# HadrienG2/grayscott

Hardware: AMD Instinct MI355X
Metric: Mcells×steps/s and achieved HBM GB/s (% of roofline), 16384² f32 grid (higher is better)
Workload: dtype f32

## Files before the change

### grayscott_amd/capi.py

```python
from __future__ import annotations

import ctypes
import os

_HERE = os.path.dirname(os.path.abspath(__file__))
LIB_PATH = os.environ.get("GS_HIP_LIBRARY") or os.path.join(_HERE, "libgs_hip.so")

GS_OK = 0
GS_ERR_INVALID = -1
GS_ERR_HIP = -2
GS_ERR_RCCL = -3
GS_ERR_NO_DEVICE = -4
GS_ERR_UNSUPPORTED = -5
GS_ERR_NOMEM = -6

GS_MATH_STRICT, GS_MATH_FUSED = 0, 1
GS_KERNEL_AUTO, GS_KERNEL_SIMPLE, GS_KERNEL_STREAM, GS_KERNEL_TB, GS_KERNEL_LDS, GS_KERNEL_TILE, GS_KERNEL_WINDOW = 0, 1, 2, 3, 4, 5, 6
GS_BOUNDARY_CLIPPED, GS_BOUNDARY_ZERO_HALO, GS_BOUNDARY_PERIODIC, GS_BOUNDARY_NEUMANN = 0, 1, 2, 3
GS_UNIQUE_ID_BYTES = 128
GS_REGION_PAIRS_MAX = 1 << 25
GS_REGION_HIST_MAX = 1 << 25
GS_REGION_SPECTRUM_MAX = 1 << 25
GS_REGION_SPECTRUM_RECORDS_MAX = 1 << 27
GS_REGION_COMPONENTS_MAX = 1 << 20
# ... 27 lines not shown
    "gs_fields_compare", "gs_members_compare", "gs_fields_copy", "gs_members_copy",
    "gs_members_set_active", "gs_members_get_active",
    "gs_members_set_noise", "gs_members_get_noise", "gs_members_clear_noise",
    "gs_fields_morphology", "gs_members_morphology",
    "gs_region_grid", "gs_fields_region_summaries", "gs_fields_region_morphology", "gs_fields_region_correlation",
    "gs_fields_region_histogram", "gs_fields_region_components", "gs_fields_region_compare", "gs_fields_region_spectrum",
    "gs_fields_correlation", "gs_members_correlation",
    "gs_spectrum_tables", "gs_fields_spectrum", "gs_members_spectrum",
    "gs_fields_components", "gs_members_components",
    "gs_field_component_list", "gs_members_component_list", "gs_component_list_view", "gs_component_list_destroy",
    "gs_fields_match", "gs_members_match", "gs_component_match_view", "gs_component_match_destroy",
    "gs_time_stats_create", "gs_time_stats_destroy", "gs_time_stats_reset", "gs_time_stats_accumulate", "gs_time_stats_samples",
    "gs_time_stats_result", "gs_time_stats_download",
    "gs_members_time_stats_create", "gs_members_time_stats_accumulate", "gs_members_time_stats_result",
    "gs_members_bundle_stats",
    "gs_ctx_quiet_stats", "gs_ctx_quiet_edge_stats",
)


class GsError(RuntimeError):

    def __init__(self, code: int, message: str):
        super().__init__(f"gs_hip error {code}: {message}")
        self.code = code
        self.message = message


class GsParams(ctypes.Structure):

    _fields_ = [
        ("w", (ctypes.c_float * 3) * 3),
# ... 157 lines not shown
        "gs_timer_start": (i32, [vp]),
        "gs_timer_stop": (i32, [vp, P(f32)]),
        "gs_ctx_info": (i32, [vp, ctypes.c_char_p, ctypes.c_size_t, P(u64)]),
        "gs_host_alloc": (i32, [P(vp), u64]),
        "gs_host_free": (i32, [vp]),
        "gs_field_download_async": (i32, [vp, vp, vp]),
        "gs_download_wait": (i32, [vp]),
        "gs_ctx_get_tuned": (i32, [vp, u64, u64, P(i32), P(i32), P(i32), P(i32)]),
        "gs_ctx_set_tuned": (i32, [vp, u64, u64, i32, i32, i32, i32]),
        "gs_ctx_comm_info": (i32, [vp, P(i32), P(i32), P(i32)]),
        "gs_field_colormap": (i32, [vp, vp, f32, vp, i32, vp]),
        "gs_ctx_stats": (i32, [vp, P(GsStats)]),
        "gs_ctx_set_pass_timing": (i32, [vp, i32]),
        "gs_ctx_quiet_stats": (i32, [vp, P(u64)]),
        "gs_ctx_quiet_edge_stats": (i32, [vp, P(u64)]),
        "gs_field_mark_written": (i32, [vp, vp]),
        "gs_rccl_selftest": (i32, [i32, u64]),
        "gs_runtime_info": (i32, [i32, ctypes.c_char_p, ctypes.c_size_t]),
        "gs_fields_place": (i32, [vp, P(vp), i32, P(f32), P(f32)]),
        "gs_debug_place_stats": (i32, [vp, P(u64), P(u64)]),
        "gs_download_wait_but": (i32, [vp, i32]),
        "gs_debug_exchange_probe_create": (i32, [i32, i32, i32, u64, P(vp)]),
        "gs_debug_exchange_probe_run": (i32, [vp, P(f32), P(f32)]),
        "gs_debug_exchange_probe_destroy": (i32, [vp]),
        "gs_ensemble_create": (i32, [vp, P(vp), u64, u64, u64]),
        "gs_ensemble_destroy": (i32, [vp, vp]),
        "gs_ensemble_shape": (i32, [vp, P(u64), P(u64), P(u64)]),
        "gs_ensemble_set_params": (i32, [vp, vp, P(GsParams), u64]),
        "gs_ensemble_seed": (i32, [vp, vp]),
        "gs_ensemble_upload": (i32, [vp, vp, u64, u64, vp, vp]),
# ... 105 lines not shown
```

### grayscott_amd/csrc/gs_api.cpp

```cpp
#include "gs_internal.h"

namespace gsi {

bool is_pow2_or_zero(float w)
{
    if (w == 0.0f) return true;
    int e = 0;
    const float m = std::frexp(std::fabs(w), &e);
    return m == 0.5f;
}

int32_t check_math(const gs_params &p, int32_t math)
{
    if (math != GS_MATH_STRICT && math != GS_MATH_FUSED)
        return fail(GS_ERR_INVALID, "unknown math flavour %d", math);
    if (math == GS_MATH_FUSED)
        for (int i = 0; i < 3; ++i)
            for (int j = 0; j < 3; ++j)
                if (!is_pow2_or_zero(p.w[i][j]))
                    return fail(GS_ERR_UNSUPPORTED,
                                "GS_MATH_FUSED needs stencil weights that are 0 or a power of two "
                                "(w[%d][%d] = %g); use GS_MATH_STRICT", i, j, (double)p.w[i][j]);
    return GS_OK;
}
// ... 169 lines not shown
                        qr.edge_skipped = sum;
                        GS_HIP(hipFree(qr.words));
                        qr.words = nullptr;
                        qr.cap = 0;
                    }
                    GS_HIP(hipMalloc(&qr.words, 3 * (size_t)q.need * sizeof(uint32_t)));
                    GS_HIP(hipMemset(qr.words, 0, 3 * (size_t)q.need * sizeof(uint32_t)));
                    qr.cap = (size_t)q.need;
                    if (!qr.skipped) {
                        GS_HIP(hipMalloc(&qr.skipped, (size_t)kQuietCounters * kQuietCounterStride * sizeof(unsigned long long)));
                        GS_HIP(hipMemset(qr.skipped, 0, (size_t)kQuietCounters * kQuietCounterStride * sizeof(unsigned long long)));
                    }
                    continue;
                }
                if (q.launched > 0) {
                    qr.launched += (uint64_t)q.launched;
                    qr.edge_launched += (uint64_t)q.edge_launched;
                    qr.passes++;
                    if (qr.mode == 3) qr.steady++;
                } else {
                    qr.refused = true;
                }
                break;
            }
            break;
        }
        e = fused ? gs_launch_tb_fused(a, fuse, stream, &name, at) : gs_launch_tb_strict(a, fuse, stream, &name, at);
        break;
    case GS_KERNEL_SIMPLE:
        e = fused ? gs_launch_simple_fused(a, stream, &name, at) : gs_launch_simple_strict(a, stream, &name, at);
// ... 443 lines not shown
                                            "set GS_RCCL_LIBRARY to the transport to use, or run one slab per process");
    }

    int ndev = 0;
    hipError_t e = hipGetDeviceCount(&ndev);
    if (e != hipSuccess || ndev == 0)
        return fail(GS_ERR_NO_DEVICE, "no HIP device available (%s)", hipGetErrorString(e));

    gs_ctx *ctx = new (std::nothrow) gs_ctx();
    if (!ctx) return fail(GS_ERR_NOMEM, "out of host memory");
    if (params) ctx->p = *params; else gs_default_params(&ctx->p);
    if (opts) ctx->o = *opts; else gs_default_options(&ctx->o);
    ctx->rank = rank;
    ctx->world = world;
    ctx->quiet.enabled = gs_env_int("GS_HIP_QUIET_UNITS", 1, 0, 1) != 0;
    int32_t st = check_math(ctx->p, ctx->o.math);
    if (st == GS_OK && ctx->o.cols_per_lane != 0 && ctx->o.cols_per_lane != 1 && ctx->o.cols_per_lane != 2 &&
        ctx->o.cols_per_lane != 4)
        st = fail(GS_ERR_INVALID, "cols_per_lane must be 0 (auto), 1, 2 or 4, not %d", ctx->o.cols_per_lane);
    if (st == GS_OK && (ctx->o.tile_shape < 0 || ctx->o.tile_shape > 3))
        st = fail(GS_ERR_INVALID, "tile_shape must be 0 (auto), 1 (32 x 64), 2 (16 x 64) or 3 (64 x 64), not %d", ctx->o.tile_shape);
    if (st == GS_OK && ctx->o.boundary != GS_BOUNDARY_CLIPPED && ctx->o.boundary != GS_BOUNDARY_ZERO_HALO &&
        ctx->o.boundary != GS_BOUNDARY_PERIODIC && ctx->o.boundary != GS_BOUNDARY_NEUMANN)
        st = fail(GS_ERR_INVALID, "unknown boundary rule %d", ctx->o.boundary);
    if (st == GS_OK && ctx->o.boundary == GS_BOUNDARY_PERIODIC) {
        if (world > 1 || n_local > 1)
            st = fail(GS_ERR_UNSUPPORTED, "the periodic boundary rule needs a single slab in a single process (got %d local "
                                          "slab(s), %d process(es))", n_local < 1 ? 1 : n_local, world);
        else if (ctx->o.kernel == GS_KERNEL_WINDOW || ctx->o.kernel == GS_KERNEL_LDS)
            st = fail(GS_ERR_UNSUPPORTED, "the periodic boundary rule has no form of the %s kernel",
// ... 77 lines not shown
}

int32_t gs_ctx_set_params(gs_ctx *ctx, const gs_params *params)
{
    if (!ctx || !params) return fail(GS_ERR_INVALID, "null argument");
    GS_TRY(check_math(*params, ctx->o.math));
    GS_TRY(resolve_window(ctx));
    ctx->p = *params;
    return GS_OK;
}

int32_t gs_step(gs_ctx *ctx, gs_field *in_u, gs_field *in_v, gs_field *out_u, gs_field *out_v)
{
    GS_TRY(check_step_fields(ctx, in_u, in_v, out_u, out_v));
    GS_TRY(check_attached_shape(ctx, in_u));
    GS_TRY(resolve_window(ctx));
    return step_impl(ctx, in_u, in_v, out_u, out_v);
}

int32_t gs_run(gs_ctx *ctx, gs_field *u0, gs_field *v0, gs_field *u1, gs_field *v1, uint64_t steps,
               int32_t *result_slot)
{
    return run_steps(ctx, u0, v0, u1, v1, steps, result_slot, true);
}

}

namespace gsi {

int32_t run_steps(gs_ctx *ctx, gs_field *u0, gs_field *v0, gs_field *u1, gs_field *v1, uint64_t steps, int32_t *result_slot,
                  bool allow_window)
{
    GS_TRY(check_step_fields(ctx, u0, v0, u1, v1));
    GS_TRY(check_attached_shape(ctx, u0));
    Run r{ctx, {u0, u1}, {v0, v1}};
    r.steps = steps;
    int fuse = 1;
    if (ctx->o.kernel == GS_KERNEL_AUTO || ctx->o.kernel == GS_KERNEL_TB || ctx->o.kernel == GS_KERNEL_TILE ||
        ctx->o.kernel == GS_KERNEL_WINDOW) {
        fuse = ctx->o.fuse_steps > 0 ? ctx->o.fuse_steps : kGhostRows;
        if (fuse > kGhostRows) fuse = kGhostRows;
        if (ctx->total_slabs() > 1 && fuse > min_slab_rows(ctx, u0)) fuse = min_slab_rows(ctx, u0);
        if (fuse < 1) fuse = 1;
    }
    const bool single = ctx->total_slabs() == 1;
    const bool mapped = ctx->attached.kind != GS_ATTACH_NONE;
    if (single && !mapped && ctx->o.kernel == GS_KERNEL_AUTO && u0->rows * u0->cols > 0 && steps > 0 &&
        u0->rows * u0->cols <= (uint64_t)kGsResidentCells) {
        SlabRt &sl = ctx->slabs[0];
// ... 81 lines not shown
    if (single && fuse > 1 && ctx->o.rows_per_block == 0 && !ctx->o.no_tune && !tuned_shape(ctx, u0, fuse))
        GS_TRY(tune_online(r, fuse));
    const int kk = tuned_shape(ctx, u0, fuse) && ctx->tuner().tuned.k > 0 && ctx->tuner().tuned.k <= fuse ? ctx->tuner().tuned.k : fuse;
    const int V = bands_for(ctx, u0, kk);
    if (ctx->o.use_graph && single && V == 1 && kk > 1) GS_TRY(replay_graph_batches(r, kk));
    gs_ctx::QuietRt &qr = ctx->quiet;
    const gs_params &pp = ctx->p;
    bool quiet = qr.enabled && single && V == 1 && !ctx->o.use_graph && !mapped && kk >= 2 && kk <= 4 &&
                 ctx->o.math == GS_MATH_STRICT && (ctx->o.boundary == GS_BOUNDARY_CLIPPED || ctx->o.boundary == GS_BOUNDARY_ZERO_HALO) &&
                 (ctx->o.kernel == GS_KERNEL_AUTO || ctx->o.kernel == GS_KERNEL_TB || ctx->o.kernel == GS_KERNEL_TILE ||
                  ctx->o.kernel == GS_KERNEL_WINDOW) &&
                 std::isfinite(pp.du) && std::isfinite(pp.dv) && std::isfinite(pp.feed) && std::isfinite(pp.kill) &&
                 std::isfinite(pp.feed + pp.kill) && std::isfinite(pp.dt);
    for (int i = 0; i < 9; ++i) quiet = quiet && std::isfinite(pp.w[i / 3][i % 3]);
    qr.refused = false;
    int quiet_pass = 0;
    const char *full_pass = nullptr;
    while (r.n < steps) {
        const int k = (steps - r.n) >= (uint64_t)kk ? kk : (int)(steps - r.n);
        if (quiet && k == kk && !qr.refused) {
            qr.mode = quiet_pass < 2 ? quiet_pass + 1 : 3;
            qr.in_slot = r.in;
            ++quiet_pass;
        }
        const int32_t st = r.advance(k == kk ? V : 1, k);
        qr.mode = 0;
        GS_TRY(st);
        if (k == kk) full_pass = ctx->last_kernel;
    }
    if (full_pass) ctx->last_kernel = full_pass;
    if (result_slot) *result_slot = r.in;
    return GS_OK;
}

}

extern "C" {

int32_t gs_sync(gs_ctx *ctx)
{
    if (!ctx) return fail(GS_ERR_INVALID, "null context");
    return sync_all(ctx);
}
// ... 93 lines not shown
int32_t gs_ctx_quiet_edge_stats(gs_ctx *ctx, uint64_t out[3])
{
    if (!ctx || !out) return fail(GS_ERR_INVALID, "null argument");
    GS_TRY(sync_all(ctx));
    out[0] = ctx->quiet.edge_launched;
    out[1] = out[2] = 0;
    if (ctx->quiet.skipped) {
        unsigned long long host[kQuietCounters * kQuietCounterStride];
        GS_HIP(hipSetDevice(ctx->slabs[0].device));
        GS_HIP(hipMemcpy(host, ctx->quiet.skipped, sizeof host, hipMemcpyDeviceToHost));
        for (int i = 0; i < kQuietCounters; ++i) out[2] += host[i * kQuietCounterStride + 2];
    }
    return gsi::quiet_edge_skips(ctx, &out[1]);
}

int32_t gs_ctx_info(const gs_ctx *ctx, char *kernel_name, size_t cap, uint64_t *launches)
{
    if (!ctx) return fail(GS_ERR_INVALID, "null context");
    if (kernel_name && cap) {
        const gs_ctx::Tuned &t = ctx->tuner().tuned;
        if (t.rpu > 0)
            std::snprintf(kernel_name, cap, "%s@%dx%d", ctx->last_kernel, t.rpu, t.split > 0 ? t.split : 1);
        else
            std::snprintf(kernel_name, cap, "%s", ctx->last_kernel);
    }
    if (launches) *launches = ctx->launches;
    return GS_OK;
}

}
// ... 1 lines not shown
```

### grayscott_amd/csrc/gs_attached.cpp

```cpp
#include "gs_internal.h"

namespace gsi {

static const char *const kKindName[GS_ATTACH_KINDS] = {"", "parameter map", "domain mask", "noise term"};
static const char *const kKindShort[GS_ATTACH_KINDS] = {"", "map", "mask", "noise"};
static const char *const kKindForm[GS_ATTACH_KINDS] = {"", "parameter-map", "domain-mask", "noise"};

static void philox2x32(uint32_t c0, uint32_t c1, uint32_t k, uint32_t out[2])
{
    for (int i = 0; i < 10; ++i) {
        const uint64_t p = (uint64_t)0xD256D193u * c0;
        c0 = (uint32_t)(p >> 32) ^ k ^ c1;
        c1 = (uint32_t)p;
        k += 0x9E3779B9u;
    }
    out[0] = c0;
    out[1] = c1;
}
uint32_t noise_key(uint64_t seed, uint64_t step)
{
    uint32_t x[2];
    philox2x32((uint32_t)step, (uint32_t)(step >> 32), (uint32_t)seed, x);
    return x[0] ^ (uint32_t)(seed >> 32);
}
// ... 58 lines not shown
    at.plane[0] = f[0];
    at.plane[1] = f[1];
    return GS_OK;
}

template <typename F>
static int32_t fill_planes(gs_ctx *ctx, gs_field *const *planes, int np, F enqueue)
{
    for (size_t i = 0; i < ctx->slabs.size(); ++i) {
        SlabRt &sl = ctx->slabs[i];
        GS_HIP(hipSetDevice(sl.device));
        GS_TRY(enqueue(i, sl, (size_t)(planes[0]->s[i].rows + 2 * kGhostRows) * planes[0]->pitch + 2 * kGuardFloats));
    }
    GS_TRY(sync_all(ctx));
    for (int j = 0; j < np; ++j) {
        planes[j]->ghost_depth = 0;
        GS_TRY(refresh_ghosts(ctx, planes[j]));
    }
    return GS_OK;
}

static int32_t copy_block(gs_field *dst, const gs_field *src, size_t i, SlabRt &sl, size_t n)
{
    GS_HIP(hipMemcpyAsync(dst->s[i].alloc, src->s[i].alloc, n * sizeof(float), hipMemcpyDeviceToDevice, sl.compute));
    return GS_OK;
}

static int32_t form_links(gs_ctx *ctx, gs_field *m)
{
    gs_field *l = ctx->attached.plane[0];
    const int32_t periodic = ctx->o.boundary == GS_BOUNDARY_PERIODIC;
// ... 92 lines not shown
```

### grayscott_amd/csrc/gs_fields.cpp

```cpp
#include <algorithm>
#include "gs_internal.h"

using namespace gsi;

namespace gsi {

int32_t plane_layout(const gs_ctx *ctx, uint64_t rows, uint64_t cols, PlaneLayout &out)
{
    const uint64_t S = (uint64_t)ctx->total_slabs();
    if (rows < S && !(rows == 0 && S == 1))
        return fail(GS_ERR_INVALID, "%llu rows cannot be split over %llu slabs",
                    (unsigned long long)rows, (unsigned long long)S);
    const int pad = ctx->o.pitch_pad > 0 ? ((ctx->o.pitch_pad + 3) / 4) * 4 : 0;
    out.pitch = (cols == 0 ? 64 : ((cols + 63) / 64) * 64) + (uint64_t)pad;
    if (out.pitch > 0x7ffffff0ull) return fail(GS_ERR_UNSUPPORTED, "too many columns");
    out.slabs.clear();
    for (size_t i = 0; i < ctx->slabs.size(); ++i) {
        const uint64_t k = (uint64_t)ctx->global_index((int)i);
        const uint64_t r0 = k * rows / S, r1 = (k + 1) * rows / S;
        if (r1 - r0 > 0x7ffffff0ull || (r1 - r0 + 2 * kGhostRows) * out.pitch > 0x7ffffff0ull * 4ull)
            return fail(GS_ERR_UNSUPPORTED, "slab too large for 32-bit row indexing");
        out.slabs.emplace_back(r0, r1 - r0);
    }
    return GS_OK;
}

}

extern "C" {

int32_t gs_field_destroy(gs_ctx *ctx, gs_field *f)
{
    if (!f) return GS_OK;
    if (ctx) (void)sync_all(ctx);
    for (size_t i = 0; i < f->s.size(); ++i)
        if (f->s[i].alloc) {
            if (ctx && i < ctx->slabs.size()) (void)hipSetDevice(ctx->slabs[i].device);
            (void)hipFree(f->s[i].alloc);
        }
    delete f;
    return GS_OK;
}

int32_t gs_field_create(gs_ctx *ctx, gs_field **out, uint64_t rows, uint64_t cols)
{
    if (!ctx || !out) return fail(GS_ERR_INVALID, "null argument");
    *out = nullptr;
    PlaneLayout layout;
    GS_TRY(plane_layout(ctx, rows, cols, layout));
// ... 31 lines not shown
{
    if (!ctx || !planes) return fail(GS_ERR_INVALID, "null argument");
    if (candidates < 1 || candidates > 124) return fail(GS_ERR_INVALID, "1 to 124 extra candidate blocks, not %d", candidates);
    if (ctx->slabs.size() != 1) return fail(GS_ERR_UNSUPPORTED, "placement by measurement is for contexts with one slab per process");
    for (int i = 0; i < 4; ++i) {
        if (!planes[i] || planes[i]->ctx != ctx) return fail(GS_ERR_INVALID, "bad plane %d", i);
        GS_TRY(same_shape(planes[0], planes[i]));
        for (int j = 0; j < i; ++j)
            if (planes[i] == planes[j]) return fail(GS_ERR_INVALID, "the four planes must be distinct");
    }
    if (first_ms) *first_ms = 0.0f;
    if (best_ms) *best_ms = 0.0f;
    const gs_field *f0 = planes[0];
    if (f0->rows == 0 || f0->cols == 0) return GS_OK;
    GS_TRY(sync_all(ctx));
    SlabRt &sl = ctx->slabs[0];
    GS_HIP(hipSetDevice(sl.device));
    const size_t pitch = (size_t)f0->pitch;
    const size_t n = (size_t)(f0->s[0].rows + 2 * kGhostRows) * pitch + 2 * kGuardFloats;
    const size_t bytes = n * sizeof(float);
    const bool trace = gs_env_int("GS_HIP_TRACE_TUNER", 0, 0, 1) != 0;
    const bool draw_all = gs_env_int("GS_HIP_PLACE_ALL", 0, 0, 1) != 0;
    std::vector<float *> blocks;
    for (int i = 0; i < 4; ++i) blocks.push_back(planes[i]->s[0].alloc);
    constexpr float kNotTimed = 1.0e9f;
    std::vector<std::vector<float>> T(4, std::vector<float>(4, 0.0f));
    int probes = 0;
    auto pair_ms = [&](int i, int j, float *ms) -> int32_t {
        float best = 0.0f;
        for (int rep = 0; rep < 3; ++rep) {
// ... 229 lines not shown
                    (unsigned long long)r0, (unsigned long long)r1, (unsigned long long)c0,
                    (unsigned long long)c1, (unsigned long long)f->rows, (unsigned long long)f->cols);
    GS_TRY(sync_all(ctx));
    for (size_t i = 0; i < f->s.size(); ++i) {
        const FieldSlab &fs = f->s[i];
        const uint64_t lo = r0 > fs.g_row0 ? r0 : fs.g_row0;
        const uint64_t hi = r1 < fs.g_row0 + fs.rows ? r1 : fs.g_row0 + fs.rows;
        if (lo >= hi || c0 >= c1) continue;
        GS_HIP(hipSetDevice(ctx->slabs[i].device));
        hipError_t e = gs_launch_fill_rect(fs.row0, f->pitch, (int32_t)(lo - fs.g_row0),
                                           (int32_t)(hi - fs.g_row0), (int32_t)c0, (int32_t)c1, value,
                                           ctx->slabs[i].compute);
        if (e != hipSuccess) return fail(GS_ERR_HIP, "fill launch failed: %s", hipGetErrorString(e));
    }
    GS_TRY(sync_all(ctx));
    f->ghost_depth = 0;
    return GS_OK;
}

int32_t gs_field_fill(gs_ctx *ctx, gs_field *f, float value)
{
    if (!f) return fail(GS_ERR_INVALID, "null field");
    return gs_field_fill_slice(ctx, f, 0, f->rows, 0, f->cols, value);
}

int32_t gs_field_finalize(gs_ctx *ctx, gs_field *f)
{
    if (!ctx || !f || f->ctx != ctx) return fail(GS_ERR_INVALID, "bad handle");
    if (f->ghost_depth == 0) GS_TRY(refresh_ghosts(ctx, f));
    return GS_OK;
}

int32_t gs_field_upload(gs_ctx *ctx, gs_field *f, const float *host)
{
    if (!ctx || !f || f->ctx != ctx) return fail(GS_ERR_INVALID, "bad argument");
    if (f->rows == 0 || f->cols == 0) return GS_OK;
    if (!host) return fail(GS_ERR_INVALID, "bad argument");
    GS_TRY(sync_all(ctx));
    const uint64_t first = f->s.front().g_row0;
    for (size_t i = 0; i < f->s.size(); ++i) {
        const FieldSlab &fs = f->s[i];
        GS_HIP(hipSetDevice(ctx->slabs[i].device));
        GS_HIP(hipMemcpy2D(fs.row0, (size_t)f->pitch * sizeof(float), host + (fs.g_row0 - first) * f->cols,
                           (size_t)f->cols * sizeof(float), (size_t)f->cols * sizeof(float), (size_t)fs.rows,
                           hipMemcpyHostToDevice));
    }
    f->ghost_depth = 0;
    return GS_OK;
}

int32_t gs_field_download(gs_ctx *ctx, gs_field *f, float *host)
{
    if (!ctx || !f || f->ctx != ctx) return fail(GS_ERR_INVALID, "bad argument");
    GS_TRY(sync_all(ctx));
    if (f->rows == 0 || f->cols == 0) return GS_OK;
    if (!host) return fail(GS_ERR_INVALID, "bad argument");
    const uint64_t first = f->s.front().g_row0;
    for (size_t i = 0; i < f->s.size(); ++i) {
        const FieldSlab &fs = f->s[i];
        GS_HIP(hipSetDevice(ctx->slabs[i].device));
        GS_HIP(hipMemcpy2D(host + (fs.g_row0 - first) * f->cols, (size_t)f->cols * sizeof(float), fs.row0,
                           (size_t)f->pitch * sizeof(float), (size_t)f->cols * sizeof(float), (size_t)fs.rows,
// ... 5 lines not shown
int32_t gs_field_device_ptr(const gs_field *f, int32_t slab, void **ptr, uint64_t *pitch, uint64_t *slab_row0,
                            uint64_t *slab_rows, int32_t *device)
{
    if (!f || slab < 0 || (size_t)slab >= f->s.size()) return fail(GS_ERR_INVALID, "bad slab index");
    if (ptr) *ptr = f->s[slab].row0;
    if (pitch) *pitch = (uint64_t)f->pitch;
    if (slab_row0) *slab_row0 = f->s[slab].g_row0;
    if (slab_rows) *slab_rows = (uint64_t)f->s[slab].rows;
    if (device) *device = f->ctx->slabs[slab].device;
    return GS_OK;
}

int32_t gs_field_mark_written(gs_ctx *ctx, gs_field *f)
{
    if (!ctx || !f || f->ctx != ctx) return fail(GS_ERR_INVALID, "bad handle");
    f->ghost_depth = 0;
    return GS_OK;
}

int32_t gs_host_alloc(void **out, uint64_t bytes)
{
    if (!out || bytes == 0) return fail(GS_ERR_INVALID, "bad argument");
    *out = nullptr;
    hipError_t e = hipHostMalloc(out, (size_t)bytes, hipHostMallocDefault);
    if (e != hipSuccess) return fail(GS_ERR_NOMEM, "hipHostMalloc(%llu) failed: %s", (unsigned long long)bytes,
                                     hipGetErrorString(e));
    return GS_OK;
}

int32_t gs_host_free(void *p)
{
// ... 230 lines not shown
```

### grayscott_amd/csrc/gs_internal.h

```cpp
#pragma once
#pragma GCC visibility push(default)
#include "../../include/gs_hip.h"
#pragma GCC visibility pop
#include "gs_kernels.h"
#include "gs_experiments.h"

#include <dlfcn.h>
#include <hip/hip_runtime.h>
#include <rccl/rccl.h>

#include <algorithm>
#include <cmath>
#include <cstdarg>
#include <cstdio>
#include <cstdlib>
#include <cstring>
#include <new>
#include <string>
#include <utility>
#include <vector>

namespace gsi {

extern thread_local std::string g_last_error;
// ... 122 lines not shown
        uint64_t rows = 0, pitch = 0;
        size_t plane_bytes = 0;
        int32_t epoch = 0;
        bool pending = false;
        bool disabled = false;
        struct Launch { gs_field *in[2], *out[2]; int steps; int32_t seq; int passes; };
        std::vector<Launch> launched;
        int32_t seq = 0;
        uint64_t fallbacks = 0;
        struct Image { gs_field *f; float *host; int32_t after_seq; int32_t factor; };
        std::vector<Image> images;
        int32_t *seen = nullptr;
    } win;
    int cu_count = 0;
    struct QuietRt {
        bool enabled = true;
        uint32_t *words = nullptr;
        size_t cap = 0;
        unsigned long long *skipped = nullptr;
        int mode = 0;
        int in_slot = 0;
        bool refused = false;
        uint64_t launched = 0, passes = 0, steady = 0;
        uint64_t edge_launched = 0;
        uint64_t edge_skipped = 0;
    } quiet;
    std::vector<struct gs_time_stats *> time_stats;
    struct Attached {
        int kind = GS_ATTACH_NONE;
        gs_field *plane[2] = {nullptr, nullptr};
// ... 33 lines not shown
    uint64_t stale_count = 0;
    uint32_t *active_list = nullptr;
    uint32_t *mirror_list = nullptr;
    bool all_active() const { return active.empty() || active_count == members; }
    std::vector<GsEnsNoise> noise;
    GsEnsNoise *noise_table = nullptr;
    uint64_t noise_clock(uint64_t m) const { return active.empty() || active[m] ? run_steps : retired_at[m]; }
};

struct gs_field {
    gs_ctx *ctx = nullptr;
    uint64_t rows = 0, cols = 0;
    int32_t pitch = 0;
    std::vector<FieldSlab> s;
    int ghost_depth = 0;
};

namespace gsi {

struct Run;

int32_t check_math(const gs_params &p, int32_t math);
int32_t same_shape(const gs_field *a, const gs_field *b);
int32_t sync_all(gs_ctx *ctx);
int32_t sync_compute(gs_ctx *ctx);
int32_t refresh_ghosts(gs_ctx *ctx, gs_field *f);
int32_t copy_row(gs_ctx *ctx, int src_slab, const float *src, int dst_slab, float *dst, size_t bytes, hipStream_t stream);
int min_slab_rows(const gs_ctx *ctx, const gs_field *f);
GsStepArgs make_args(const gs_ctx *ctx, const gs_field *in_u, const gs_field *in_v,
                     const gs_field *out_u, const gs_field *out_v, int i, int fuse);
int32_t join_bands(gs_ctx *ctx, hipStream_t stream);
int bands_for(const gs_ctx *ctx, const gs_field *f, int fuse);
int32_t step_bands(gs_ctx *ctx, gs_field *in_u, gs_field *in_v, gs_field *out_u, gs_field *out_v, int fuse, int V);
// ... 69 lines not shown
```

### grayscott_amd/csrc/gs_observe.cpp

```cpp
#include "gs_internal.h"
#include "gs_components_merge.h"
#include "gs_match_merge.h"

#include <cstdlib>
#include <cstring>
#include <memory>

using namespace gsi;

struct gs_component_list {
    uint64_t planes = 0;
    std::vector<uint64_t> offsets;
    std::vector<gs_component_record> records;
};

struct gs_component_match {
    gs_component_list before, after;
    std::vector<uint64_t> offsets;
    std::vector<gs_component_overlap> overlaps;
};

namespace gsi {

int32_t ensure_scratch(gs_ctx *ctx, int i, size_t bytes, const char *what)
// ... 864 lines not shown
            for (int32_t q = 0; q < p; ++q)
                if (dst[p] && dst[p] == dst[q]) return fail(GS_ERR_INVALID, "fields %d and %d: one target named twice", q, p);
        }
    GS_TRY(check_planes(ctx, dst, n, src));
    const gs_field *f0 = dst[0];
    if (f0->rows == 0 || f0->cols == 0) return GS_OK;
    const size_t pitch_bytes = (size_t)f0->pitch * sizeof(float), row_bytes = (size_t)f0->cols * sizeof(float);
    for (size_t i = 0; i < ctx->slabs.size(); ++i) {
        SlabRt &sl = ctx->slabs[i];
        GS_HIP(hipSetDevice(sl.device));
        for (int32_t p = 0; p < n; ++p)
            GS_HIP(hipMemcpy2DAsync(dst[p]->s[i].row0, pitch_bytes, src[p]->s[i].row0, pitch_bytes, row_bytes,
                                    (size_t)f0->s[i].rows, hipMemcpyDeviceToDevice, sl.compute));
    }
    GS_TRY(sync_compute(ctx));
    for (int32_t p = 0; p < n; ++p) dst[p]->ghost_depth = 0;
    return GS_OK;
}

int32_t gs_members_copy(gs_ctx *ctx, gs_ensemble *dst, gs_ensemble *src, uint64_t first, uint64_t count)
{
    if (!ctx) return fail(GS_ERR_INVALID, "null argument");
    if (dst && dst == src) return fail(GS_ERR_INVALID, "an ensemble would be copied onto itself");
    GS_TRY(check_members(ctx, dst, first, count, src, true));
    const size_t cells = (size_t)(dst->rows * dst->cols), off = (size_t)first * cells, bytes = (size_t)count * cells * sizeof(float);
    if (bytes == 0) return GS_OK;
    SlabRt &sl = ctx->slabs[0];
    GS_HIP(hipSetDevice(sl.device));
    GS_HIP(hipMemcpyAsync(dst->u[dst->cur] + off, src->u[src->cur] + off, bytes, hipMemcpyDeviceToDevice, sl.compute));
    GS_HIP(hipMemcpyAsync(dst->v[dst->cur] + off, src->v[src->cur] + off, bytes, hipMemcpyDeviceToDevice, sl.compute));
    mark_members_written(dst, first, count);
// ... 791 lines not shown
```

### grayscott_amd/csrc/gs_time_stats.cpp

```cpp
#include "gs_internal.h"
#include "gs_plane_scan.h"

using namespace gsi;

struct gs_time_stats {
    gs_ctx *ctx = nullptr;
    uint64_t rows = 0, cols = 0;
    int32_t n = 0;
    uint32_t groups = 0;
    float t[4] = {0, 0, 0, 0};
    uint32_t flip[4] = {0, 0, 0, 0};
    uint64_t samples = 0;
    bool members = false;
    uint64_t first = 0, count = 0;
    struct Slab {
        void *alloc = nullptr;
        GsTstatAcc acc{};
        int64_t rows = 0;
        uint64_t g_row0 = 0;
    };
    std::vector<Slab> s;
    int64_t pitch = 0;
};

// ... 290 lines not shown
    if (!out) return fail(GS_ERR_INVALID, "null argument");
    GS_TRY(check_object(ctx, ts, false));
    GS_TRY(check_result(ts, plane, which));
    if (out->ctx != ctx) return fail(GS_ERR_INVALID, "result field of another context");
    if (out->rows != ts->rows || out->cols != ts->cols || (int64_t)out->pitch != ts->pitch)
        return fail(GS_ERR_INVALID, "result field of [%llu, %llu], time statistics of [%llu, %llu]", (unsigned long long)out->rows,
                    (unsigned long long)out->cols, (unsigned long long)ts->rows, (unsigned long long)ts->cols);
    GS_TRY(sync_all(ctx));
    for (size_t i = 0; i < ts->s.size(); ++i) {
        if (!ts->s[i].alloc) continue;
        GS_HIP(hipSetDevice(ctx->slabs[i].device));
        GS_HIP(gs_launch_tstat_result(which, plane, ts->s[i].acc, ts->pitch, ts->s[i].rows, (int32_t)ts->cols, ts->samples,
                                      out->s[i].row0, ctx->slabs[i].compute));
    }
    GS_TRY(sync_compute(ctx));
    out->ghost_depth = 0;
    return GS_OK;
}

int32_t gs_members_time_stats_result(gs_ctx *ctx, gs_time_stats *ts, int32_t species, int32_t which, float *host)
{
    if (!host) return fail(GS_ERR_INVALID, "null argument");
    GS_TRY(check_object(ctx, ts, true));
    GS_TRY(check_result(ts, species, which));
    GS_TRY(sync_all(ctx));
    const gs_time_stats::Slab &sl = ts->s[0];
    const size_t bytes = (size_t)sl.rows * (size_t)ts->cols * sizeof(float);
    GS_TRY(ensure_scratch(ctx, 0, bytes, "time statistics"));
    SlabRt &rt = ctx->slabs[0];
    GS_HIP(hipSetDevice(rt.device));
    float *dev = static_cast<float *>(rt.scratch);
// ... 37 lines not shown
```

### grayscott_amd/csrc/gs_window.cpp

```cpp
#include "gs_internal.h"

namespace gsi {

std::vector<GsWindowDesc> plan_windows(const gs_ctx *ctx, uint64_t rows, uint64_t cols, int want_rpw, int want_k, int *rpw_out, int *k_out)
{
    const bool cheap = (fast_of(ctx) & 3) == 3 && ctx->o.math == GS_MATH_STRICT && gs_env_int("GS_HIP_EDGE_KINDS", 1, 0, 1) != 0;
    return plan_windows(ctx->cu_count, ctx->o.boundary == GS_BOUNDARY_ZERO_HALO, cheap, rows, cols, want_rpw, want_k, rpw_out, k_out);
}

std::vector<GsWindowDesc> plan_windows(int cu_count, bool zero_halo, bool cheap, uint64_t rows, uint64_t cols, int want_rpw, int want_k,
                                       int *rpw_out, int *k_out)
{
    if (want_k <= 0) {
        for (int k : {8, 6, 4, 2}) {
            std::vector<GsWindowDesc> plan = plan_windows(cu_count, zero_halo, cheap, rows, cols, want_rpw, k, rpw_out, k_out);
            if (!plan.empty()) return plan;
        }
        return std::vector<GsWindowDesc>();
    }
    std::vector<GsWindowDesc> plan;
    if (cu_count <= 0 || rows == 0 || cols == 0 || rows > 0x7fffff || cols > 0x7fffff) return plan;
    const int k = want_k;
    if (k < 2 || k > 8 || (k & 1)) return plan;
    const long wo = 128 - 2 * k;
// ... 124 lines not shown
    w.disabled = true;
    w.fallbacks++;
    for (const auto &l : launched) {
        if (l.seq < gave_up) continue;
        ctx->launches -= 1;
        ctx->passes -= (uint64_t)l.passes;
        ctx->steps_done -= (uint64_t)l.steps;
        int32_t slot = 0;
        GS_TRY(run_steps(ctx, l.in[0], l.in[1], l.out[0], l.out[1], (uint64_t)l.steps, &slot, false));
        if (slot != 1) {
            for (int sp = 0; sp < 2; ++sp) {
                const gs_field *src = l.in[sp];
                gs_field *dst = l.out[sp];
                const size_t bytes = (size_t)src->s[0].rows * (size_t)src->pitch * sizeof(float);
                GS_HIP(hipMemcpyAsync(dst->s[0].row0, src->s[0].row0, bytes, hipMemcpyDeviceToDevice, sl.compute));
                dst->ghost_depth = src->ghost_depth;
            }
        }
        for (const auto &im : images)
            if (im.after_seq == l.seq) {
                GS_HIP(hipStreamSynchronize(sl.compute));
                GS_HIP(hipStreamSynchronize(sl.copy));
                GS_HIP(hipStreamSynchronize(sl.copy2));
                if (im.factor > 1) {
                    GS_TRY(fetch_reduced(ctx, im.f, im.factor, im.host));
                    continue;
                }
                const FieldSlab &fs = im.f->s[0];
                GS_HIP(hipMemcpy2D(im.host, (size_t)im.f->cols * sizeof(float), fs.row0, (size_t)im.f->pitch * sizeof(float),
                                   (size_t)im.f->cols * sizeof(float), (size_t)fs.rows, hipMemcpyDeviceToHost));
// ... 109 lines not shown
```

### grayscott_amd/simulation.py

```python
from __future__ import annotations

import ctypes
import math
import os
from dataclasses import dataclass, field
from typing import Callable, List, Optional, Sequence, Tuple

import numpy as np

from . import capi
from .capi import GsError

STENCIL_WEIGHTS = ((0.25, 0.5, 0.25), (0.5, 0.0, 0.5), (0.25, 0.5, 0.25))

STENCILS = {
    "oono-puri": STENCIL_WEIGHTS,
    "5points": ((0.0, 1.0, 0.0), (1.0, 0.0, 1.0), (0.0, 1.0, 0.0)),
    "patrakarttunen": ((1 / 6, 4 / 6, 1 / 6), (4 / 6, 0.0, 4 / 6), (1 / 6, 4 / 6, 1 / 6)),
    "pretty": ((1.0, 1.0, 1.0), (1.0, 1.0, 1.0), (1.0, 1.0, 1.0)),
}


@dataclass
class Parameters:
# ... 127 lines not shown

    def stats(self) -> dict:
        st = capi.GsStats()
        capi.check(self._lib.gs_ctx_stats(self.handle, ctypes.byref(st)))
        return {name: getattr(st, name) for name, _ in capi.GsStats._fields_ if name != "reserved"}

    def quiet_stats(self) -> Tuple[int, int, int, int]:
        out = (ctypes.c_uint64 * 4)()
        capi.check(self._lib.gs_ctx_quiet_stats(self.handle, out))
        return int(out[0]), int(out[1]), int(out[2]), int(out[3])

    def quiet_edge_stats(self) -> Tuple[int, int, int]:
        out = (ctypes.c_uint64 * 3)()
        capi.check(self._lib.gs_ctx_quiet_edge_stats(self.handle, out))
        return int(out[0]), int(out[1]), int(out[2])

    def set_pass_timing(self, passes: int) -> None:
        capi.check(self._lib.gs_ctx_set_pass_timing(self.handle, passes))

    def info(self) -> Tuple[str, int]:
        buf = ctypes.create_string_buffer(64)
        n = ctypes.c_uint64(0)
        capi.check(self._lib.gs_ctx_info(self.handle, buf, 64, ctypes.byref(n)))
        return buf.value.decode(), int(n.value)

    def close(self) -> None:
        if self._h:
            self._lib.gs_ctx_destroy(self._h)
            self._h = ctypes.c_void_p()

# ... 2094 lines not shown
```

### include/grayscott_hip.hpp

```cpp
#pragma once
#include "gs_hip.h"

#include <array>
#include <cmath>
#include <cstddef>
#include <memory>
#include <stdexcept>
#include <string>
#include <utility>
#include <vector>

namespace gs {

using Precision = float;

struct HipError : std::runtime_error {
    int32_t code;
    HipError(int32_t c, const std::string &m)
        : std::runtime_error("gs_hip error " + std::to_string(c) + ": " + m), code(c) {}
};

inline void check(int32_t status)
{
    if (status != GS_OK) throw HipError(status, gs_last_error());
// ... 340 lines not shown
    ~HipContext() { gs_ctx_destroy(ctx_); }
    int32_t place_candidates() const { return place_candidates_; }
    HipContext(const HipContext &) = delete;
    HipContext &operator=(const HipContext &) = delete;
    gs_ctx *get() const { return ctx_; }
    void sync() const { check(gs_sync(ctx_)); }
    void download_wait() const { check(gs_download_wait(ctx_)); }
    void download_wait_but(int32_t in_flight) const { check(gs_download_wait_but(ctx_, in_flight)); }
    gs_stats stats() const
    {
        gs_stats st;
        check(gs_ctx_stats(ctx_, &st));
        return st;
    }
    void set_pass_timing(int32_t passes) const { check(gs_ctx_set_pass_timing(ctx_, passes)); }


  private:
    gs_ctx *ctx_ = nullptr;
    int32_t place_candidates_ = 0;
};
using Context = std::shared_ptr<HipContext>;

using Shape = std::array<std::size_t, 2>;
using Range = std::pair<std::size_t, std::size_t>;

class HipConcentration {
  public:
    static HipConcentration default_(Context &c, Shape s) { return HipConcentration(c, s); }
    static HipConcentration zeros(Context &c, Shape s) { return HipConcentration(c, s); }
// ... 899 lines not shown
```

### include/gs_hip.h

```cpp
#ifndef GS_HIP_H
#define GS_HIP_H

#include <stddef.h>
#include <stdint.h>

#ifdef __cplusplus
extern "C" {
#endif

#define GS_ABI_VERSION 4

typedef enum gs_status {
    GS_OK = 0,
    GS_ERR_INVALID = -1,
    GS_ERR_HIP = -2,
    GS_ERR_RCCL = -3,
    GS_ERR_NO_DEVICE = -4,
    GS_ERR_UNSUPPORTED = -5,
    GS_ERR_NOMEM = -6
} gs_status;

typedef struct gs_params {
    float w[3][3];
    float du;
// ... 125 lines not shown
    uint64_t passes;
    uint64_t steps;
    uint64_t launches;
    uint64_t ghost_refreshes;
    uint64_t timed_passes;
    float halo_ms;
    float interior_ms;
    float halo_exposed_ms;
    float reserved;
    uint64_t window_fallbacks;
} gs_stats;
int32_t gs_ctx_stats(gs_ctx *ctx, gs_stats *out);
int32_t gs_ctx_set_pass_timing(gs_ctx *ctx, int32_t passes);
int32_t gs_ctx_quiet_stats(gs_ctx *ctx, uint64_t out[4]);
int32_t gs_ctx_quiet_edge_stats(gs_ctx *ctx, uint64_t out[3]);

int32_t gs_ctx_info(const gs_ctx *ctx, char *kernel_name, size_t cap, uint64_t *launches);

typedef struct gs_ensemble gs_ensemble;
int32_t gs_ensemble_create(gs_ctx *ctx, gs_ensemble **out, uint64_t members, uint64_t rows, uint64_t cols);
int32_t gs_ensemble_destroy(gs_ctx *ctx, gs_ensemble *e);
int32_t gs_ensemble_shape(const gs_ensemble *e, uint64_t *members, uint64_t *rows, uint64_t *cols);
int32_t gs_ensemble_set_params(gs_ctx *ctx, gs_ensemble *e, const gs_params *params, uint64_t count);
int32_t gs_ensemble_seed(gs_ctx *ctx, gs_ensemble *e);
int32_t gs_ensemble_upload(gs_ctx *ctx, gs_ensemble *e, uint64_t first, uint64_t count, const float *u, const float *v);
int32_t gs_ensemble_download(gs_ctx *ctx, gs_ensemble *e, uint64_t first, uint64_t count, int32_t species, float *host);
int32_t gs_ensemble_run(gs_ctx *ctx, gs_ensemble *e, uint64_t steps);

int32_t gs_members_set_active(gs_ctx *ctx, gs_ensemble *e, uint64_t first, uint64_t count, const uint8_t *active);
int32_t gs_members_get_active(gs_ctx *ctx, gs_ensemble *e, uint64_t first, uint64_t count, uint8_t *active, uint64_t *steps_taken,
// ... 158 lines not shown
```

### rust/compute_hip/src/ffi.rs

```rust
#![allow(non_camel_case_types)]

use std::os::raw::{c_char, c_void};

pub const GS_OK: i32 = 0;
pub const GS_UNIQUE_ID_BYTES: usize = 128;

#[repr(C)]
#[derive(Copy, Clone, Debug)]
pub struct gs_params {
    pub w: [[f32; 3]; 3],
    pub du: f32,
    pub dv: f32,
    pub feed: f32,
    pub kill: f32,
    pub dt: f32,
}

#[repr(C)]
#[derive(Copy, Clone, Debug, Default)]
pub struct gs_options {
    pub math: i32,
    pub kernel: i32,
    pub rows_per_block: i32,
    pub fuse_steps: i32,
// ... 377 lines not shown
    pub fn gs_members_time_stats_accumulate(ctx: *mut gs_ctx, ts: *mut gs_time_stats, e: *mut gs_ensemble, stamp: u32) -> i32;
    pub fn gs_members_time_stats_result(ctx: *mut gs_ctx, ts: *mut gs_time_stats, species: i32, which: i32, host: *mut f32) -> i32;
    pub fn gs_members_bundle_stats(
        ctx: *mut gs_ctx,
        e: *mut gs_ensemble,
        first: u64,
        count: u64,
        span: u64,
        which: *const i32,
        n: i32,
        thresholds: *const f32,
        above: *const i32,
        out: *const *mut gs_ensemble,
        out_first: u64,
    ) -> i32;
}
```

Measured before the change: 5.006 million.

## Carry quiet-unit skip state across gs_run calls when fields are unchanged

Adds a carry record of the quiet-unit tracking state (field handles, per-field write counters, geometry) at the end of each gs_run. The next run with the same buffers, unmodified fields and the same geometry resumes in steady quiet-skip mode instead of restarting the detection warm-up passes. A write counter is added to fields and bumped by every mutation path so stale carries are invalidated. The aim is to skip more quiet work in the early passes of repeated short runs, at the risk of wrongly skipping cells if some mutation path misses the counter.

```diff
diff --git a/grayscott_amd/capi.py b/grayscott_amd/capi.py
--- a/grayscott_amd/capi.py
+++ b/grayscott_amd/capi.py
@@ -65,7 +65,7 @@
     "gs_time_stats_result", "gs_time_stats_download",
     "gs_members_time_stats_create", "gs_members_time_stats_accumulate", "gs_members_time_stats_result",
     "gs_members_bundle_stats",
-    "gs_ctx_quiet_stats", "gs_ctx_quiet_edge_stats",
+    "gs_ctx_quiet_stats", "gs_ctx_quiet_edge_stats", "gs_ctx_quiet_carry_stats",
 )
 
 
@@ -253,6 +253,7 @@
         "gs_ctx_set_pass_timing": (i32, [vp, i32]),
         "gs_ctx_quiet_stats": (i32, [vp, P(u64)]),
         "gs_ctx_quiet_edge_stats": (i32, [vp, P(u64)]),
+        "gs_ctx_quiet_carry_stats": (i32, [vp, P(u64)]),
         "gs_field_mark_written": (i32, [vp, vp]),
         "gs_rccl_selftest": (i32, [i32, u64]),
         "gs_runtime_info": (i32, [i32, ctypes.c_char_p, ctypes.c_size_t]),
diff --git a/grayscott_amd/csrc/gs_api.cpp b/grayscott_amd/csrc/gs_api.cpp
--- a/grayscott_amd/csrc/gs_api.cpp
+++ b/grayscott_amd/csrc/gs_api.cpp
@@ -207,6 +207,8 @@
                     continue;
                 }
                 if (q.launched > 0) {
+                    qr.ran = true;
+                    qr.need = q.need;
                     qr.launched += (uint64_t)q.launched;
                     qr.edge_launched += (uint64_t)q.edge_launched;
                     qr.passes++;
@@ -680,6 +682,7 @@
     ctx->rank = rank;
     ctx->world = world;
     ctx->quiet.enabled = gs_env_int("GS_HIP_QUIET_UNITS", 1, 0, 1) != 0;
+    ctx->quiet.carry_enabled = gs_env_int("GS_HIP_QUIET_CARRY", 1, 0, 1) != 0;
     int32_t st = check_math(ctx->p, ctx->o.math);
     if (st == GS_OK && ctx->o.cols_per_lane != 0 && ctx->o.cols_per_lane != 1 && ctx->o.cols_per_lane != 2 &&
         ctx->o.cols_per_lane != 4)
@@ -787,6 +790,7 @@
 {
     GS_TRY(check_step_fields(ctx, in_u, in_v, out_u, out_v));
     GS_TRY(check_attached_shape(ctx, in_u));
+    ctx->quiet.carry.valid = 0;
     GS_TRY(resolve_window(ctx));
     return step_impl(ctx, in_u, in_v, out_u, out_v);
 }
@@ -806,6 +810,8 @@
 {
     GS_TRY(check_step_fields(ctx, u0, v0, u1, v1));
     GS_TRY(check_attached_shape(ctx, u0));
+    const gs_ctx::QuietRt::Carry carried = ctx->quiet.carry;
+    ctx->quiet.carry.valid = 0;
     Run r{ctx, {u0, u1}, {v0, v1}};
     r.steps = steps;
     int fuse = 1;
@@ -917,19 +923,56 @@
                  std::isfinite(pp.feed + pp.kill) && std::isfinite(pp.dt);
     for (int i = 0; i < 9; ++i) quiet = quiet && std::isfinite(pp.w[i / 3][i % 3]);
     qr.refused = false;
+    gs_ctx::QuietRt::Carry now;
+    if (quiet) {
+        const GsStepArgs a = make_args(ctx, u0, v0, u1, v1, 0, kk);
+        now.rows = a.rows; now.cols = a.cols; now.pitch = a.pitch; now.rpu = a.rows_per_unit; now.k = kk; now.cpl = a.cpl;
+        now.fast = a.fast; now.edge_kinds = a.edge_kinds; now.boundary = a.zero_halo;
+    }
     int quiet_pass = 0;
+    qr.slot_xor = 0;
+    if (quiet && qr.carry_enabled && carried.valid > 0 && r.n == 0 && qr.words && carried.need <= (int64_t)qr.cap &&
+        carried.same_geometry(now)) {
+        const int a = carried.newest;
+        if (u0 == carried.u[a] && v0 == carried.v[a] && u1 == carried.u[1 - a] && v1 == carried.v[1 - a] &&
+            u0->writes == carried.writes[a][0] && v0->writes == carried.writes[a][1] &&
+            u1->writes == carried.writes[1 - a][0] && v1->writes == carried.writes[1 - a][1]) {
+            quiet_pass = carried.valid < 2 ? carried.valid : 2;
+            qr.slot_xor = a;
+        }
+    }
+    const int opened = quiet_pass;
+    bool counted = false, last_ran = false;
     const char *full_pass = nullptr;
     while (r.n < steps) {
         const int k = (steps - r.n) >= (uint64_t)kk ? kk : (int)(steps - r.n);
+        qr.ran = false;
         if (quiet && k == kk && !qr.refused) {
             qr.mode = quiet_pass < 2 ? quiet_pass + 1 : 3;
-            qr.in_slot = r.in;
+            qr.in_slot = r.in ^ qr.slot_xor;
             ++quiet_pass;
         }
         const int32_t st = r.advance(k == kk ? V : 1, k);
         qr.mode = 0;
         GS_TRY(st);
+        last_ran = qr.ran;
+        if (qr.ran && !counted) {
+            counted = true;
+            if (opened >= 2) qr.carried++;
+            else if (opened == 0) qr.restarted++;
+        }
         if (k == kk) full_pass = ctx->last_kernel;
+    }
+    if (quiet && qr.carry_enabled && last_ran && !qr.refused && allow_window) {
+        now.valid = quiet_pass < 2 ? quiet_pass : 2;
+        now.newest = r.in ^ qr.slot_xor;
+        for (int i = 0; i < 2; ++i) {
+            const int ws = i ^ qr.slot_xor;
+            now.u[ws] = r.u[i]; now.v[ws] = r.v[i];
+            now.writes[ws][0] = r.u[i]->writes; now.writes[ws][1] = r.v[i]->writes;
+        }
+        now.need = qr.need;
+        qr.carry = now;
     }
     if (full_pass) ctx->last_kernel = full_pass;
     if (result_slot) *result_slot = r.in;
@@ -1053,6 +1096,14 @@
     return gsi::quiet_edge_skips(ctx, &out[1]);
 }
 
+int32_t gs_ctx_quiet_carry_stats(gs_ctx *ctx, uint64_t out[2])
+{
+    if (!ctx || !out) return fail(GS_ERR_INVALID, "null argument");
+    out[0] = ctx->quiet.carried;
+    out[1] = ctx->quiet.restarted;
+    return GS_OK;
+}
+
 int32_t gs_ctx_info(const gs_ctx *ctx, char *kernel_name, size_t cap, uint64_t *launches)
 {
     if (!ctx) return fail(GS_ERR_INVALID, "null context");
diff --git a/grayscott_amd/csrc/gs_attached.cpp b/grayscott_amd/csrc/gs_attached.cpp
--- a/grayscott_amd/csrc/gs_attached.cpp
+++ b/grayscott_amd/csrc/gs_attached.cpp
@@ -96,7 +96,7 @@
     }
     GS_TRY(sync_all(ctx));
     for (int j = 0; j < np; ++j) {
-        planes[j]->ghost_depth = 0;
+        mark_written(planes[j]);
         GS_TRY(refresh_ghosts(ctx, planes[j]));
     }
     return GS_OK;
diff --git a/grayscott_amd/csrc/gs_fields.cpp b/grayscott_amd/csrc/gs_fields.cpp
--- a/grayscott_amd/csrc/gs_fields.cpp
+++ b/grayscott_amd/csrc/gs_fields.cpp
@@ -33,6 +33,7 @@
 {
     if (!f) return GS_OK;
     if (ctx) (void)sync_all(ctx);
+    if (ctx && ctx->quiet.carry.holds(f)) ctx->quiet.carry.valid = 0;
     for (size_t i = 0; i < f->s.size(); ++i)
         if (f->s[i].alloc) {
             if (ctx && i < ctx->slabs.size()) (void)hipSetDevice(ctx->slabs[i].device);
@@ -94,6 +95,7 @@
     const gs_field *f0 = planes[0];
     if (f0->rows == 0 || f0->cols == 0) return GS_OK;
     GS_TRY(sync_all(ctx));
+    for (int i = 0; i < 4; ++i) planes[i]->writes++;
     SlabRt &sl = ctx->slabs[0];
     GS_HIP(hipSetDevice(sl.device));
     const size_t pitch = (size_t)f0->pitch;
@@ -353,7 +355,7 @@
         if (e != hipSuccess) return fail(GS_ERR_HIP, "fill launch failed: %s", hipGetErrorString(e));
     }
     GS_TRY(sync_all(ctx));
-    f->ghost_depth = 0;
+    mark_written(f);
     return GS_OK;
 }
 
@@ -384,7 +386,7 @@
                            (size_t)f->cols * sizeof(float), (size_t)f->cols * sizeof(float), (size_t)fs.rows,
                            hipMemcpyHostToDevice));
     }
-    f->ghost_depth = 0;
+    mark_written(f);
     return GS_OK;
 }
 
@@ -420,7 +422,7 @@
 int32_t gs_field_mark_written(gs_ctx *ctx, gs_field *f)
 {
     if (!ctx || !f || f->ctx != ctx) return fail(GS_ERR_INVALID, "bad handle");
-    f->ghost_depth = 0;
+    mark_written(f);
     return GS_OK;
 }
 
diff --git a/grayscott_amd/csrc/gs_internal.h b/grayscott_amd/csrc/gs_internal.h
--- a/grayscott_amd/csrc/gs_internal.h
+++ b/grayscott_amd/csrc/gs_internal.h
@@ -160,6 +160,25 @@
     } win;
     int cu_count = 0;
     struct QuietRt {
+        struct Carry {
+            int valid = 0;
+            int newest = 0;
+            gs_field *u[2] = {nullptr, nullptr}, *v[2] = {nullptr, nullptr};
+            uint64_t writes[2][2] = {{0, 0}, {0, 0}};
+            int32_t rows = 0, cols = 0, pitch = 0, rpu = 0, k = 0, cpl = 0, fast = 0, edge_kinds = 0, boundary = 0;
+            int64_t need = 0;
+            bool same_geometry(const Carry &o) const
+            {
+                return rows == o.rows && cols == o.cols && pitch == o.pitch && rpu == o.rpu && k == o.k && cpl == o.cpl &&
+                       fast == o.fast && edge_kinds == o.edge_kinds && boundary == o.boundary;
+            }
+            bool holds(const gs_field *f) const { return valid > 0 && (f == u[0] || f == u[1] || f == v[0] || f == v[1]); }
+        } carry;
+        bool carry_enabled = true;
+        uint64_t carried = 0, restarted = 0;
+        int slot_xor = 0;
+        int64_t need = 0;
+        bool ran = false;
         bool enabled = true;
         uint32_t *words = nullptr;
         size_t cap = 0;
@@ -223,9 +242,16 @@
     int32_t pitch = 0;
     std::vector<FieldSlab> s;
     int ghost_depth = 0;
+    uint64_t writes = 0;
 };
 
 namespace gsi {
+
+inline void mark_written(gs_field *f)
+{
+    f->ghost_depth = 0;
+    f->writes++;
+}
 
 struct Run;
 
diff --git a/grayscott_amd/csrc/gs_observe.cpp b/grayscott_amd/csrc/gs_observe.cpp
--- a/grayscott_amd/csrc/gs_observe.cpp
+++ b/grayscott_amd/csrc/gs_observe.cpp
@@ -902,7 +902,7 @@
                                     (size_t)f0->s[i].rows, hipMemcpyDeviceToDevice, sl.compute));
     }
     GS_TRY(sync_compute(ctx));
-    for (int32_t p = 0; p < n; ++p) dst[p]->ghost_depth = 0;
+    for (int32_t p = 0; p < n; ++p) mark_written(dst[p]);
     return GS_OK;
 }
 
diff --git a/grayscott_amd/csrc/gs_time_stats.cpp b/grayscott_amd/csrc/gs_time_stats.cpp
--- a/grayscott_amd/csrc/gs_time_stats.cpp
+++ b/grayscott_amd/csrc/gs_time_stats.cpp
@@ -328,7 +328,7 @@
                                       out->s[i].row0, ctx->slabs[i].compute));
     }
     GS_TRY(sync_compute(ctx));
-    out->ghost_depth = 0;
+    mark_written(out);
     return GS_OK;
 }
 
diff --git a/grayscott_amd/csrc/gs_window.cpp b/grayscott_amd/csrc/gs_window.cpp
--- a/grayscott_amd/csrc/gs_window.cpp
+++ b/grayscott_amd/csrc/gs_window.cpp
@@ -162,6 +162,7 @@
                 gs_field *dst = l.out[sp];
                 const size_t bytes = (size_t)src->s[0].rows * (size_t)src->pitch * sizeof(float);
                 GS_HIP(hipMemcpyAsync(dst->s[0].row0, src->s[0].row0, bytes, hipMemcpyDeviceToDevice, sl.compute));
+                mark_written(dst);
                 dst->ghost_depth = src->ghost_depth;
             }
         }
diff --git a/grayscott_amd/simulation.py b/grayscott_amd/simulation.py
--- a/grayscott_amd/simulation.py
+++ b/grayscott_amd/simulation.py
@@ -165,6 +165,11 @@
         out = (ctypes.c_uint64 * 3)()
         capi.check(self._lib.gs_ctx_quiet_edge_stats(self.handle, out))
         return int(out[0]), int(out[1]), int(out[2])
+
+    def quiet_carry_stats(self) -> Tuple[int, int]:
+        out = (ctypes.c_uint64 * 2)()
+        capi.check(self._lib.gs_ctx_quiet_carry_stats(self.handle, out))
+        return int(out[0]), int(out[1])
 
     def set_pass_timing(self, passes: int) -> None:
         capi.check(self._lib.gs_ctx_set_pass_timing(self.handle, passes))
diff --git a/include/grayscott_hip.hpp b/include/grayscott_hip.hpp
--- a/include/grayscott_hip.hpp
+++ b/include/grayscott_hip.hpp
@@ -378,6 +378,12 @@
         return st;
     }
     void set_pass_timing(int32_t passes) const { check(gs_ctx_set_pass_timing(ctx_, passes)); }
+    std::pair<uint64_t, uint64_t> quiet_carry_stats() const
+    {
+        uint64_t out[2] = {0, 0};
+        check(gs_ctx_quiet_carry_stats(ctx_, out));
+        return {out[0], out[1]};
+    }
 
 
   private:
diff --git a/include/gs_hip.h b/include/gs_hip.h
--- a/include/gs_hip.h
+++ b/include/gs_hip.h
@@ -163,6 +163,7 @@
 int32_t gs_ctx_set_pass_timing(gs_ctx *ctx, int32_t passes);
 int32_t gs_ctx_quiet_stats(gs_ctx *ctx, uint64_t out[4]);
 int32_t gs_ctx_quiet_edge_stats(gs_ctx *ctx, uint64_t out[3]);
+int32_t gs_ctx_quiet_carry_stats(gs_ctx *ctx, uint64_t out[2]);
 
 int32_t gs_ctx_info(const gs_ctx *ctx, char *kernel_name, size_t cap, uint64_t *launches);
 
diff --git a/rust/compute_hip/src/ffi.rs b/rust/compute_hip/src/ffi.rs
--- a/rust/compute_hip/src/ffi.rs
+++ b/rust/compute_hip/src/ffi.rs
@@ -415,4 +415,5 @@
         out: *const *mut gs_ensemble,
         out_first: u64,
     ) -> i32;
-}
+    pub fn gs_ctx_quiet_carry_stats(ctx: *mut gs_ctx, out: *mut u64) -> i32;
+}
```

After: 4.935 million. -1.4%, worse.
